# d-f/nylon-amt

Measured on AMD Instinct MI355X. Metric: training clips/sec (128-frame x 256-bin), higher is better.
Workload: dtype f16x3 (split fp16 / bf16 operand pairs, three bf16-rate MFMA passes per product, fp32 accumulate; tensors that flow between kernels are fp32 (attention q/k/v as fp16 hi+lo pairs), the copies SAVED only for the backward -- FFN hidden, its gradient, pre-LayerNorm sums -- are bf16); 1 GPU; paper-size hFT-Transformer training step (d=256, ff=512, 3+3 layers, 4 heads), batch 8 clips/GPU, dropout 0.10, forward+loss+backward+Adam; global_batch=8, frames=128, bins=256, parallelism=dp1, precision_mode=x3

## Files before the change

include/hftt_hip.h:

```cpp
#ifndef HFTT_HIP_H
#define HFTT_HIP_H
#include <stdint.h>
#ifdef __cplusplus
extern "C" {
#endif

#define HFTT_ABI_VERSION 8

int hftt_abi_version(void);
int hftt_build_options(void);
const char* hftt_last_error(void);
int hftt_device_cus(void);


typedef struct {
  int64_t src_off;
  int64_t dst_off;
  int32_t rows, cols, src_ld, dst_ld;
  int32_t kind;
  int32_t pad;
} hftt_prep_entry;
int hftt_prep_weights(const float* params, uint16_t* wbf, float* wf32, float* fdst,
                      const hftt_prep_entry* table_dev, int n_entries, void* stream);
int hftt_prep_weights_x3(const float* params, uint16_t* whi, uint16_t* wlo, float* fdst,
// ... 150 lines not shown
  float* dr; float* dr_drop;
  float drop_p; uint32_t drop_site; uint64_t drop_seed;
  float* ws;
  uint32_t drop_bf16;
  uint32_t io_flags;
} hftt_ln_bwd_desc;
#define HFTT_LNB_DY_BF16 1u
#define HFTT_LNB_DR_BF16 2u
#define HFTT_LNB_R_BF16 4u
int32_t hftt_ln_bwd_wgs(int32_t M);
int hftt_ln_bwd(const hftt_ln_bwd_desc* d, void* stream);
int hftt_ln_bwd_reduce(const float* ws, int32_t n_wg, int32_t N, float* dgamma, float* dbeta, float beta, void* stream);

#define HFTT_TE_X_BF16 1u
#define HFTT_TE_Y_BF16 2u
#define HFTT_TE_M_BF16 4u
int hftt_time_embed_fwd(const float* x, const float* pos, float* y, int32_t B, int32_t T, int32_t Nn, int32_t d,
                        float scale, float drop_p, uint32_t site, uint64_t seed, uint32_t io_flags, void* stream);
int hftt_time_embed_bwd(const float* dy, float* dx, float* dym, int32_t B, int32_t T, int32_t Nn, int32_t d,
                        float scale, float drop_p, uint32_t site, uint64_t seed, int32_t accumulate, uint32_t io_flags, void* stream);
int hftt_dropout_bwd(float* g, int64_t n, float drop_p, uint32_t site, uint64_t seed, uint32_t bf16, void* stream);
int hftt_colsum(const float* x, int64_t rows, int64_t n, int64_t ld, float* out, float beta, float* ws, uint32_t x_bf16, void* stream);
int64_t hftt_colsum_ws_bytes(int64_t rows, int64_t n);
int hftt_heads_split(const float* logits, int64_t ldl, float* onset, float* offset, float* mpe, float* velocity,
                     int32_t B, int32_t T, int32_t Nn, int32_t V, int32_t time_major, void* stream);
int hftt_heads_split_bwd(const float* p_onset, const float* p_offset, const float* p_mpe,
                         const float* d_onset, const float* d_offset, const float* d_mpe, const float* d_velocity,
                         float* dlogits, int64_t ldl, int32_t B, int32_t T, int32_t Nn, int32_t V, int32_t time_major,
                         void* stream);

typedef struct {
  int64_t n;
  int32_t V; int32_t pad;
  const float* prob[6];
  const float* vel[2];
  const float* label_onset; const float* label_offset; const float* label_mpe; const int64_t* label_velocity;
  float weight_A, weight_B, grad_scale; float pad2;
  float* d_prob[6]; float* d_vel[2];
  float* loss_out;
  float* ws;
} hftt_loss_desc;
int64_t hftt_loss_ws_bytes(int64_t n);
int hftt_loss(const hftt_loss_desc* d, void* stream);

int hftt_adam_step(float* p, const float* g, float* m, float* v, int64_t n, int32_t step,
                   double lr, double beta1, double beta2, double eps, double grad_scale, void* stream);
// ... 237 lines not shown
```

nylon-amt_amd/csrc/elementwise.hip:

```cpp
#include "hftt_common.h"
#include "x3_common.h"
#include "hftt_launch.h"
#include "../../include/hftt_hip.h"
#include <math.h>

namespace {

template <int E>
__device__ __forceinline__ void x3_split1(float x, uint16_t& hi, uint16_t& lo) {
  unsigned h, l;
  x3_split2_checked<E>(x, 0.f, h, l);
  hi = (uint16_t)(h & 0xFFFFu); lo = (uint16_t)(l & 0xFFFFu);
}

__global__ void prep_weights_kernel(const float* __restrict__ params, uint16_t* __restrict__ wbf, float* __restrict__ wf32,
                                    float* __restrict__ fdst, const hftt_prep_entry* __restrict__ table) {
  const hftt_prep_entry e = table[blockIdx.x];
  const long total = (long)e.rows * e.cols;
  for (long i = (long)blockIdx.y * blockDim.x + threadIdx.x; i < total; i += (long)gridDim.y * blockDim.x) {
    const int r = (int)(i / e.cols), c = (int)(i % e.cols);
    const float x = params[e.src_off + (long)r * e.src_ld + c];
    if (e.kind == 2) {
      fdst[e.dst_off + (long)r * e.dst_ld + c] = x;
    } else {
// ... 514 lines not shown
  for (long i = (long)blockIdx.x * blockDim.x + threadIdx.x; i < n4; i += (long)gridDim.x * blockDim.x) {
    const float4 a = hftt_load4(gbuf, bf, i * 4);
    float v[4] = {a.x, a.y, a.z, a.w};
    const uint32_t k4 = hftt_keep_quad(seed, site, (uint64_t)i, thr);
#pragma unroll
    for (int e = 0; e < 4; e++) v[e] = ((k4 >> e) & 1u) ? v[e] * inv_keep : 0.f;
    hftt_store4(gbuf, bf, i * 4, v[0], v[1], v[2], v[3]);
  }
}

constexpr int CS_SPLITS = 16;
__global__ void colsum_stage1_kernel(const float* __restrict__ x, long rows, long n, long ld, float* __restrict__ ws, uint32_t bf) {
  const long j = (long)blockIdx.x * blockDim.x + threadIdx.x;
  if (j >= n) return;
  const int sp = blockIdx.y;
  const long per = (rows + CS_SPLITS - 1) / CS_SPLITS;
  const long r0 = sp * per;
  long r1 = r0 + per; if (r1 > rows) r1 = rows;
  float acc = 0.f;
  if (bf) { for (long r = r0; r < r1; r++) acc += bf2f(reinterpret_cast<const unsigned short*>(x)[r * ld + j]); }
  else { for (long r = r0; r < r1; r++) acc += x[r * ld + j]; }
  ws[(long)sp * n + j] = acc;
}
__global__ void colsum_stage2_kernel(const float* __restrict__ ws, long n, float* __restrict__ out, float beta) {
  const long j = (long)blockIdx.x * blockDim.x + threadIdx.x;
  if (j >= n) return;
  float acc = 0.f;
#pragma unroll
  for (int s = 0; s < CS_SPLITS; s++) acc += ws[(long)s * n + j];
  out[j] = (beta != 0.f) ? (out[j] * beta + acc) : acc;
}

__device__ __forceinline__ float sigmoidf_(float x) { return 1.0f / (1.0f + expf(-x)); }

__global__ void heads_split_kernel(const float* __restrict__ logits, long ldl, float* __restrict__ onset, float* __restrict__ offset,
                                   float* __restrict__ mpe, float* __restrict__ velocity, int B, int T, int Nn, int V, int time_major) {
  const int v4 = V / 4;
  const long total = (long)B * T * Nn * v4;
  for (long i = (long)blockIdx.x * blockDim.x + threadIdx.x; i < total; i += (long)gridDim.x * blockDim.x) {
    const int c4 = (int)(i % v4);
    const long s = i / v4;
    long o = s;
    if (time_major) {
      const int t = (int)(s % T);
      const int n = (int)((s / T) % Nn);
      const int b = (int)(s / ((long)T * Nn));
// ... 276 lines not shown
  return hftt_launch<ln_bwd_reduce_kernel>("ln_bwd_reduce", dim3((2 * N + 15) / 16), dim3(256), 0, (hipStream_t)stream, ws, n_wg, N, dgamma, dbeta, beta);
}

extern "C" int hftt_time_embed_fwd(const float* x, const float* pos, float* y, int32_t B, int32_t T, int32_t Nn, int32_t d,
                                   float scale, float drop_p, uint32_t site, uint64_t seed, uint32_t io_flags, void* stream) {
  HFTT_REQUIRE(x && pos && y && d % 4 == 0, "time_embed_fwd: bad arguments");
  return hftt_launch<time_embed_fwd_kernel>("time_embed_fwd", dim3(grid_for((long)B * T * Nn * (d / 4), 256, 8192)), dim3(256), 0, (hipStream_t)stream,
                                                              x, pos, y, B, T, Nn, d, scale, drop_p, site, seed, io_flags);
}
extern "C" int hftt_time_embed_bwd(const float* dy, float* dx, float* dym, int32_t B, int32_t T, int32_t Nn, int32_t d,
                                   float scale, float drop_p, uint32_t site, uint64_t seed, int32_t accumulate, uint32_t io_flags, void* stream) {
  HFTT_REQUIRE(dy && dx && d % 4 == 0, "time_embed_bwd: bad arguments");
  return hftt_launch<time_embed_bwd_kernel>("time_embed_bwd", dim3(grid_for((long)B * T * Nn * (d / 4), 256, 8192)), dim3(256), 0, (hipStream_t)stream,
                                                              dy, dx, dym, B, T, Nn, d, scale, drop_p, site, seed, accumulate, io_flags);
}
extern "C" int hftt_dropout_bwd(float* g, int64_t n, float drop_p, uint32_t site, uint64_t seed, uint32_t bf16, void* stream) {
  HFTT_REQUIRE(g && n > 0 && n % 4 == 0 && drop_p >= 0.f && drop_p < 1.f && ((uintptr_t)g & 15) == 0, "dropout_bwd: bad arguments (n %% 4 == 0, 16-byte aligned)");
  if (drop_p == 0.f) return 0;
  return hftt_launch<dropout_bwd_kernel>("dropout_bwd", dim3(grid_for(n / 4, 256, 8192)), dim3(256), 0, (hipStream_t)stream, g, (long)n, drop_p, site, seed, bf16);
}
extern "C" int64_t hftt_colsum_ws_bytes(int64_t rows, int64_t n) { (void)rows; return (int64_t)CS_SPLITS * n * 4; }
extern "C" int hftt_colsum(const float* x, int64_t rows, int64_t n, int64_t ld, float* out, float beta, float* ws, uint32_t x_bf16, void* stream) {
  HFTT_REQUIRE(x && out && ws && rows > 0 && n > 0 && ld >= n, "colsum: bad arguments");
  if (int rc = hftt_launch<colsum_stage1_kernel>("colsum(1)", dim3((unsigned)((n + 255) / 256), CS_SPLITS), dim3(256), 0, (hipStream_t)stream, x, (long)rows, (long)n, (long)ld, ws, x_bf16)) return rc;
  return hftt_launch<colsum_stage2_kernel>("colsum(2)", dim3((unsigned)((n + 255) / 256)), dim3(256), 0, (hipStream_t)stream, ws, (long)n, out, beta);
}
extern "C" int hftt_heads_split(const float* logits, int64_t ldl, float* onset, float* offset, float* mpe, float* velocity,
                                int32_t B, int32_t T, int32_t Nn, int32_t V, int32_t time_major, void* stream) {
  HFTT_REQUIRE(logits && onset && offset && mpe && velocity, "heads_split: null operand");
  HFTT_REQUIRE(V % 4 == 0 && ldl % 4 == 0 && ldl >= V + 3, "heads_split: V=%d / ldl=%ld unsupported", V, (long)ldl);
  return hftt_launch<heads_split_kernel>("heads_split", dim3(grid_for((long)B * T * Nn * (V / 4), 256, 8192)), dim3(256), 0, (hipStream_t)stream,
                                                        logits, (long)ldl, onset, offset, mpe, velocity, B, T, Nn, V, time_major);
}
extern "C" int hftt_heads_split_bwd(const float* p_onset, const float* p_offset, const float* p_mpe,
                                    const float* d_onset, const float* d_offset, const float* d_mpe, const float* d_velocity,
                                    float* dlogits, int64_t ldl, int32_t B, int32_t T, int32_t Nn, int32_t V, int32_t time_major, void* stream) {
  HFTT_REQUIRE(p_onset && p_offset && p_mpe && d_onset && d_offset && d_mpe && d_velocity && dlogits, "heads_split_bwd: null operand");
  HFTT_REQUIRE(V % 4 == 0 && ldl % 4 == 0 && ldl >= V + 4, "heads_split_bwd: V=%d / ldl=%ld unsupported", V, (long)ldl);
  return hftt_launch<heads_split_bwd_kernel>("heads_split_bwd", dim3(grid_for((long)B * T * Nn * (ldl / 4), 256, 8192)), dim3(256), 0, (hipStream_t)stream,
                                                                p_onset, p_offset, p_mpe, d_onset, d_offset, d_mpe, d_velocity, dlogits, (long)ldl, B, T, Nn, V, time_major);
}

extern "C" int64_t hftt_loss_ws_bytes(int64_t n) { (void)n; return (int64_t)LOSS_WGS * 8 * 4; }
extern "C" int hftt_loss(const hftt_loss_desc* d, void* stream) {
  HFTT_REQUIRE(d && d->n > 0 && d->V > 0 && d->V <= 256, "loss: bad shape");
  for (int i = 0; i < 6; i++) HFTT_REQUIRE(d->prob[i] != nullptr, "loss: null probability tensor %d", i);
  HFTT_REQUIRE(d->vel[0] && d->vel[1] && d->label_onset && d->label_offset && d->label_mpe && d->label_velocity && d->loss_out && d->ws, "loss: null operand");
  int wgs = (int)((d->n + 3) / 4);
// ... 20 lines not shown
```

nylon-amt_amd/csrc/gemm_nt.hip:

```cpp
#include <type_traits>
#include "hftt_common.h"
#include "x3_common.h"
#include "hftt_launch.h"
#include "../../include/hftt_hip.h"

namespace {

__device__ __forceinline__ float4 load_gate4(const float* gate, bool bf, long off) {
  if (bf) {
    const uint2 u = *reinterpret_cast<const uint2*>(reinterpret_cast<const unsigned short*>(gate) + off);
    return make_float4(bf2f(u.x & 0xFFFFu), bf2f(u.x >> 16), bf2f(u.y & 0xFFFFu), bf2f(u.y >> 16));
  }
  return *reinterpret_cast<const float4*>(gate + off);
}
__device__ __forceinline__ void store_c4(float* C, bool bf, long off, float a, float b, float c, float d) {
  if (bf) {
    uint2 u;
    u.x = f2bf(a) | ((unsigned)f2bf(b) << 16); u.y = f2bf(c) | ((unsigned)f2bf(d) << 16);
    *reinterpret_cast<uint2*>(reinterpret_cast<unsigned short*>(C) + off) = u;
  } else {
    *reinterpret_cast<float4*>(C + off) = make_float4(a, b, c, d);
  }
}

// ... 371 lines not shown
      float s = 0.f;
#pragma unroll
      for (int e = 0; e < VPL; e++) s += v[e];
      const float mean = wave_sum(s) * (1.0f / BN);
      float q = 0.f;
#pragma unroll
      for (int e = 0; e < VPL; e++) { const float dlt = v[e] - mean; q += dlt * dlt; }
      const float var = wave_sum(q) * (1.0f / BN);
      const float rstd = 1.0f / sqrtf(var + 1e-5f);
#pragma unroll
      for (int e = 0; e < VPL; e++) {
        const int col = lane * VPL + e;
        if (g.pre_ln_out != nullptr) g.pre_ln_out[row * g.ldc + col] = v[e];
        g.C[row * g.ldc + col] = (v[e] - mean) * rstd * g.ln_gamma[col] + g.ln_beta[col];
      }
      if (lane == 0) {
        if (g.ln_mean != nullptr) g.ln_mean[row] = mean;
        if (g.ln_rstd != nullptr) g.ln_rstd[row] = rstd;
      }
    }
  }
}

template <int BM_, typename CH>
__device__ __forceinline__ void load_a_block(const hftt_gemm_nt_desc g, const long m0, unsigned short* As, const int RSA) {
  constexpr bool ABF = std::is_same<CH, uint4>::value;
  using T = typename std::conditional<ABF, unsigned short, float>::type;
  constexpr int E = 16 / sizeof(T);
  const T* A = reinterpret_cast<const T*>(g.A);
  const int cpr = g.K / E;
  const int total = BM_ * cpr;
  const int drow = 512 / cpr, dch = 512 - drow * cpr;
  int row = threadIdx.x / cpr, ch = threadIdx.x - row * cpr;
  for (int base = 0; base < total; base += 512 * 8) {
    CH v[8];
    int rr[8], cc[8];
#pragma unroll
    for (int u = 0; u < 8; u++) {
      rr[u] = row; cc[u] = ch;
      const bool in = row < BM_;
      const long grow = m0 + row;
      const long gr = (in && grow < g.M) ? grow : (m0 < g.M ? m0 : 0);
      const CH t = *reinterpret_cast<const CH*>(A + gr * g.lda + ch * E);
      if constexpr (ABF) v[u] = (in && grow < g.M) ? t : make_uint4(0u, 0u, 0u, 0u);
      else v[u] = (in && grow < g.M) ? t : make_float4(0.f, 0.f, 0.f, 0.f);
      row += drow; ch += dch;
      if (ch >= cpr) { ch -= cpr; row++; }
    }
#pragma unroll
    for (int u = 0; u < 8; u++)
      if (rr[u] < BM_) {
        unsigned short* dst = ABF ? As + rr[u] * RSA + (cc[u] << 3) : As + rr[u] * RSA + ((cc[u] >> 1) << 3) + (cc[u] & 1) * 4;
        if constexpr (ABF) {
          *reinterpret_cast<uint4*>(dst) = v[u];
        } else {
          typedef __bf16 bf4_t __attribute__((ext_vector_type(4)));
          const f32x4 fv = {v[u].x, v[u].y, v[u].z, v[u].w};
          *reinterpret_cast<uint2*>(dst) = __builtin_bit_cast(uint2, __builtin_convertvector(fv, bf4_t));
        }
      }
  }
}

template <int BM_, int MODE, bool EW = false, int PF = 1>
__global__ __launch_bounds__(512) __attribute__((amdgpu_waves_per_eu(4, MODE == 0 ? 8 : 4))) void gemm_nt_as1_kernel(const hftt_gemm_nt_desc g) {
  constexpr int BN = 256;
  constexpr int WM = (BM_ == 32) ? 1 : 2;
  constexpr int WN = 8 / WM;
  constexpr int TN = BN / (32 * WN);
  static_assert(BM_ == 32 * WM, "one 32-row MFMA tile per wave row");
  constexpr int RSW = 40;
  constexpr int W_ELEMS = BN * RSW;
  constexpr int WCH = 2;
  constexpr int STAGE_LD = BN + 4;
  static_assert(MODE != 2 || BM_ * STAGE_LD * 4 <= 2 * W_ELEMS * 2, "stage must fit the weight ring");
  extern __shared__ __attribute__((aligned(16))) unsigned char smem[];
  const int K = g.K;
  const int RSA = K + 8;
  unsigned short* As = reinterpret_cast<unsigned short*>(smem);
  unsigned short* Ws = As + BM_ * RSA;
  float* stage = (MODE == 2) ? reinterpret_cast<float*>(Ws) : reinterpret_cast<float*>(smem);

  const int tid = threadIdx.x, lane = tid & 63, wave = tid >> 6;
// ... 147 lines not shown
          const float v = fmaxf(acc[j][r] + bv, lo_clamp) * g.out_scale;
          acc[j][r] = 0.f;
          if (MODE != 0) {
            sp[rofs * STAGE_LD] = v;
          } else {
            if (full || m0 + rb0 + rofs < g.M) cp[(long)rofs * g.ldc] = v;
          }
        }
      }
      if (MODE != 0) {
        __syncthreads();
        row_pass<BM_ / 8, (BM_ / 8 < 4 ? BM_ / 8 : 4), true, true>(g, m0, n0, stage, STAGE_LD, true, thr, inv_keep);
        if (s + 1 < steps) {
          __syncthreads();
          wstore(wr[0], buf ^ 1);
        }
      }
    }
    __syncthreads();
    s++;
  }
}

template <int BM_, int MODE, bool EW = false, int PF = 1>
int launch_nt_as1(const hftt_gemm_nt_desc& d, hipStream_t st) {
  int lds = (BM_ * (d.K + 8) + 2 * 256 * 40) * 2;
  const int stage = BM_ * 260 * 4;
  if (MODE == 1 && stage > lds) lds = stage;
  dim3 grid((unsigned)((d.M + BM_ - 1) / BM_), 1, 1);
  return hftt_launch<gemm_nt_as1_kernel<BM_, MODE, EW, PF>>("gemm_nt", grid, dim3(512), lds, st, d);
}

template <int BN, int PREC, bool LN>
int launch_nt(const hftt_gemm_nt_desc& d, hipStream_t st) {
  using Cfg = NtCfg<BN, PREC>;
  int lds = Cfg::LOOP_BYTES;
  if ((LN || (Cfg::X3M && BN == 256)) && Cfg::STAGE_BYTES > lds) lds = Cfg::STAGE_BYTES;
  const int n_pad = ((d.N + 63) / 64) * 64;
  dim3 grid((unsigned)((d.M + BM - 1) / BM), (unsigned)((n_pad + BN - 1) / BN), 1);
  return hftt_launch<gemm_nt_kernel<BN, PREC, LN>>("gemm_nt", grid, dim3(512), lds, st, d);
}

template <int PREC>
int dispatch_nt(const hftt_gemm_nt_desc& d, hipStream_t st) {
  const int n_pad = ((d.N + 63) / 64) * 64;
  if (d.ln_gamma != nullptr) {
// ... 39 lines not shown
  return dispatch_nt<1>(d, st);
}

}

extern "C" int hftt_gemm_nt(const hftt_gemm_nt_desc* d, void* stream) {
  HFTT_REQUIRE(d != nullptr, "gemm_nt: null descriptor");
  HFTT_REQUIRE(d->M > 0 && d->N > 0 && d->K > 0, "gemm_nt: bad shape M=%d N=%d K=%d", d->M, d->N, d->K);
  HFTT_REQUIRE(d->K % 32 == 0, "gemm_nt: K=%d must be a multiple of 32", d->K);
  HFTT_REQUIRE((d->io_flags & ~HFTT_NT_A_HI) == 0 || d->npass == 1, "gemm_nt: bf16-stored operands need npass == 1");
  HFTT_REQUIRE(!(d->io_flags & HFTT_NT_A_HI) || d->npass == 4, "gemm_nt: HFTT_NT_A_HI goes with npass == 4");
  HFTT_REQUIRE(!(d->io_flags & HFTT_NT_C_BF16) || d->ln_gamma == nullptr, "gemm_nt: a bf16 C cannot be combined with LayerNorm");
  HFTT_REQUIRE(d->lda % ((d->io_flags & HFTT_NT_A_BF16) ? 8 : 4) == 0, "gemm_nt: lda=%ld breaks 16-byte row alignment", (long)d->lda);
  HFTT_REQUIRE(((uintptr_t)d->A & 15) == 0 && ((uintptr_t)d->W & 15) == 0, "gemm_nt: A/W must be 16-byte aligned");
  HFTT_REQUIRE(d->npass >= 1 && d->npass <= 4, "gemm_nt: npass must be 1 (bf16), 2 (split fp16), 3 (fp32) or 4 (split bf16)");
  HFTT_REQUIRE((d->npass != 2 && d->npass != 4) || d->W_lo != nullptr, "gemm_nt: the split modes need the lo weight plane (W_lo)");
  HFTT_REQUIRE(d->A != nullptr && d->W != nullptr && d->C != nullptr, "gemm_nt: null operand");
  HFTT_REQUIRE(d->add_table == nullptr || d->add_mod > 0, "gemm_nt: add_mod must be > 0");
  HFTT_REQUIRE(d->residual == nullptr || d->res_mod > 0, "gemm_nt: res_mod must be > 0");
  HFTT_REQUIRE(d->drop_p >= 0.f && d->drop_p < 1.f, "gemm_nt: drop_p out of range");
  HFTT_REQUIRE(d->ln_gamma == nullptr || (d->ln_beta != nullptr && d->ldc == d->N), "gemm_nt: LN needs beta and ldc == N");
  hipStream_t st = reinterpret_cast<hipStream_t>(stream);
  if (d->npass == 3) return dispatch_nt<3>(*d, st);
  if (d->npass == 2) return dispatch_nt<2>(*d, st);
#ifdef HFTT_GRAD_HI_BUILD
  if (d->npass == 4 && (d->io_flags & HFTT_NT_A_HI)) return dispatch_nt<5>(*d, st);
#else
  HFTT_REQUIRE(!(d->io_flags & HFTT_NT_A_HI), "gemm_nt: this library was built without the gradient-rounding option (HFTT_BUILD_GRAD_HI=1 python nylon-amt_amd/build.py)");
#endif
  if (d->npass == 4) return dispatch_nt<4>(*d, st);
  return dispatch_nt_bf16(*d, st);
}
```

nylon-amt_amd/hftt_hip/_capi.py:

```python
from __future__ import annotations

import ctypes as C
import os

_HERE = os.path.dirname(os.path.abspath(__file__))
_LIB_NAME = 'libhftt_hip_g' if os.environ.get('HFTT_BUILD_GRAD_HI') == '1' else 'libhftt_hip'
LIB_PATH = os.environ.get('HFTT_LIB_PATH') or os.path.join(_HERE, '..', 'lib', _LIB_NAME + '.so')

c_f32p = C.c_void_p
c_u16p = C.c_void_p


class PrepEntry(C.Structure):
    _fields_ = [('src_off', C.c_int64), ('dst_off', C.c_int64),
                ('rows', C.c_int32), ('cols', C.c_int32), ('src_ld', C.c_int32), ('dst_ld', C.c_int32),
                ('kind', C.c_int32), ('pad', C.c_int32)]


class GemmNtDesc(C.Structure):
    _fields_ = [('M', C.c_int32), ('N', C.c_int32), ('K', C.c_int32), ('npass', C.c_int32),
                ('A', c_f32p), ('lda', C.c_int64),
                ('W', C.c_void_p), ('io_flags', C.c_uint32), ('debug', C.c_uint32),
                ('bias', c_f32p),
                ('C', c_f32p), ('ldc', C.c_int64),
# ... 271 lines not shown
    'hftt_x3_strip_pack': (C.c_int, [c_f32p, c_u16p, C.c_void_p, C.c_int, C.c_int, C.c_void_p]),
    'hftt_strip_linear': (C.c_int, [C.POINTER(StripDesc), C.c_void_p]),
    'hftt_ffn_res_ln_fwd': (C.c_int, [C.POINTER(FfnDesc), C.c_void_p]),
    'hftt_ffn_bwd_dx': (C.c_int, [C.POINTER(FfnDesc), C.c_void_p]),
    'hftt_attn_out_ffn_fwd': (C.c_int, [C.POINTER(StripDesc), C.POINTER(FfnDesc), C.c_void_p]),
    'hftt_gemm_tn_ws_bytes': (C.c_int64, [C.c_int32, C.c_int32, C.c_int32]),
    'hftt_gemm_tn': (C.c_int, [C.POINTER(GemmTnDesc), C.c_void_p]),
    'hftt_attn_fwd': (C.c_int, [C.POINTER(AttnDesc), C.c_void_p]),
    'hftt_attn_bwd': (C.c_int, [C.POINTER(AttnDesc), C.c_void_p]),
    'hftt_x3_to_planes': (C.c_int, [c_f32p, C.c_int64, c_f32p, C.c_int64, C.c_int32, C.c_int32, C.c_void_p]),
    'hftt_embed_fold_fwd': (C.c_int, [C.POINTER(FoldDesc), C.c_void_p]),
    'hftt_embed_fold_bwd': (C.c_int, [C.POINTER(FoldDesc), C.c_void_p]),
    'hftt_im2win': (C.c_int, [c_f32p, c_f32p, C.c_int32, C.c_int32, C.c_int32, C.c_int32, C.c_int32, C.c_void_p]),
    'hftt_ln_bwd_wgs': (C.c_int32, [C.c_int32]),
    'hftt_ln_bwd': (C.c_int, [C.POINTER(LnBwdDesc), C.c_void_p]),
    'hftt_ln_bwd_reduce': (C.c_int, [c_f32p, C.c_int32, C.c_int32, c_f32p, c_f32p, C.c_float, C.c_void_p]),
    'hftt_time_embed_fwd': (C.c_int, [c_f32p, c_f32p, c_f32p, C.c_int32, C.c_int32, C.c_int32, C.c_int32,
                                      C.c_float, C.c_float, C.c_uint32, C.c_uint64, C.c_uint32, C.c_void_p]),
    'hftt_time_embed_bwd': (C.c_int, [c_f32p, c_f32p, c_f32p, C.c_int32, C.c_int32, C.c_int32, C.c_int32,
                                      C.c_float, C.c_float, C.c_uint32, C.c_uint64, C.c_int32, C.c_uint32, C.c_void_p]),
    'hftt_dropout_bwd': (C.c_int, [c_f32p, C.c_int64, C.c_float, C.c_uint32, C.c_uint64, C.c_uint32, C.c_void_p]),
    'hftt_colsum': (C.c_int, [c_f32p, C.c_int64, C.c_int64, C.c_int64, c_f32p, C.c_float, c_f32p, C.c_uint32, C.c_void_p]),
    'hftt_colsum_ws_bytes': (C.c_int64, [C.c_int64, C.c_int64]),
    'hftt_heads_split': (C.c_int, [c_f32p, C.c_int64, c_f32p, c_f32p, c_f32p, c_f32p,
                                   C.c_int32, C.c_int32, C.c_int32, C.c_int32, C.c_int32, C.c_void_p]),
    'hftt_heads_split_bwd': (C.c_int, [c_f32p, c_f32p, c_f32p, c_f32p, c_f32p, c_f32p, c_f32p, c_f32p, C.c_int64,
                                       C.c_int32, C.c_int32, C.c_int32, C.c_int32, C.c_int32, C.c_void_p]),
    'hftt_loss_ws_bytes': (C.c_int64, [C.c_int64]),
    'hftt_loss': (C.c_int, [C.POINTER(LossDesc), C.c_void_p]),
    'hftt_adam_step': (C.c_int, [c_f32p, c_f32p, c_f32p, c_f32p, C.c_int64, C.c_int32,
                                 C.c_double, C.c_double, C.c_double, C.c_double, C.c_double, C.c_void_p]),
    'hftt_logmel': (C.c_int, [C.POINTER(LogmelDesc), C.c_void_p]),
    'hftt_resample': (C.c_int, [C.POINTER(ResampleDesc), C.c_void_p]),
    'hftt_stitch': (C.c_int, [C.POINTER(StitchDesc), C.c_void_p]),
    'hftt_notes_ws_bytes': (C.c_int64, [C.c_int64, C.c_int32]),
    'hftt_notes_decode': (C.c_int, [C.POINTER(NotesDesc), C.c_void_p]),
    'hftt_clip_windows': (C.c_int, [C.POINTER(ClipWindowsDesc), C.c_void_p]),
    'hftt_notes_seg_ws_bytes': (C.c_int64, [C.c_int64, C.c_int32, C.c_int32]),
    'hftt_notes_decode_seg': (C.c_int, [C.POINTER(NotesSegDesc), C.c_void_p]),
    'hftt_notes_stream_state_bytes': (C.c_int64, [C.c_int32, C.c_int32]),
    'hftt_notes_stream_step': (C.c_int, [C.POINTER(NotesStreamDesc), C.c_void_p]),
    'hftt_labels_render': (C.c_int, [C.POINTER(LabelsDesc), C.c_void_p]),
    'hftt_clip_logmel': (C.c_int, [C.POINTER(ClipLogmelDesc), C.c_void_p]),
    'hftt_clip_logmel_warp': (C.c_int, [C.POINTER(ClipLogmelWarpDesc), C.c_void_p]),
    'hftt_wave_warp': (C.c_int, [C.POINTER(WaveWarpDesc), C.c_void_p]),
    'hftt_labels_render_warp': (C.c_int, [C.POINTER(LabelsWarpDesc), C.c_void_p]),
# ... 43 lines not shown
```

nylon-amt_amd/hftt_hip/engine.py:

```python
from __future__ import annotations

import ctypes as C
import math
import os

import torch

from . import _capi
from ._capi import FoldDesc, LossDesc, PrepEntry, StripPackEntry, check, lib
from .layout import PRECISION_NPASS, Options, WeightLayout, _align, flat_offsets, model_dims, precision_modes
from .plan import PlanBuilder, attn_fwd8_takes


def keep_scale(p):
    if not p > 0.0:
        return 1.0
    import numpy as np
    kk = (1.0 - float(np.float32(p))) * 256.0 + 0.5
    thr = 256 if kk >= 256.0 else (0 if kk <= 0.0 else int(kk))
    return float(np.float32(256.0) / np.float32(thr)) if thr > 0 else 0.0


def _table(entry_type, rows):
    return torch.frombuffer(bytearray(bytes((entry_type * len(rows))(*[entry_type(*r) for r in rows]))), dtype=torch.uint8)
# ... 210 lines not shown
            elif fn == 'heads':
                logits, tm = args
                o = outs[5:9] if tm else outs[0:4]
                rc = L.hftt_heads_split(logits, self.NHp, o[0].data_ptr(), o[1].data_ptr(), o[2].data_ptr(), o[3].data_ptr(), B, T, N, V, tm, stream)
            elif fn == 'heads_bwd':
                side, dlog, tm = args
                b = ws['bufs']
                po = outs[5:8] if tm else outs[0:3]
                rc = L.hftt_heads_split_bwd(po[0].data_ptr(), po[1].data_ptr(), po[2].data_ptr(),
                                            b['d.onset_' + side].data_ptr(), b['d.offset_' + side].data_ptr(), b['d.mpe_' + side].data_ptr(),
                                            b['d.velocity_' + side].data_ptr(), dlog, self.NHp, B, T, N, V, tm, stream)
            elif fn == 'time_embed':
                x, pos, y, site, iof = args
                rc = L.hftt_time_embed_fwd(x, pos, y, B, T, N, d, math.sqrt(d), p, site, seed, iof, stream)
            elif fn == 'time_embed_bwd':
                dy, dx, dym, site, iof = args
                rc = L.hftt_time_embed_bwd(dy, dx, dym, B, T, N, d, math.sqrt(d), p, site, seed, 1, iof, stream)
            elif fn == 'colsum':
                x, rows, n, ld, out, beta, wsp, xbf = args
                rc = L.hftt_colsum(x, rows, n, ld, out, beta, wsp, xbf, stream)
            elif fn == 'dropout_bwd':
                g, n, site, gbf = args
                rc = L.hftt_dropout_bwd(g, n, p, site, seed, gbf, stream) if p > 0.0 else 0
            else:
                raise _capi.HfttError('unknown plan op %s' % fn)
            if prof is not None:
                prof.end()
            if rc != 0:
                check(rc, name)

    def _patch(self, ws, p, seed):
        inv_keep = keep_scale(p)
        for dsc in ws['drop']:
            dsc.drop_p = p
            dsc.drop_seed = seed
        for dsc in ws.get('gate_descs', ()):
            dsc.gate_scale = inv_keep

    def forward(self, spec, training=False, outputs=None, save=None):
        if spec.dim() != 3 or spec.shape[1] != self.F or spec.shape[2] != self.W:
            raise _capi.HfttError('input_spec must be [B, %d, %d], got %s' % (self.F, self.W, tuple(spec.shape)))
        if not self.is_bound():
            raise _capi.HfttError('engine parameters are not bound (call bind first)')
        B = spec.shape[0]
        with torch.cuda.device(self.device):
            return self._forward(spec, B, training, outputs, save)
# ... 104 lines not shown
```

nylon-amt_amd/hftt_hip/plan.py:

```python
import ctypes as C
import math
import os

import torch

from . import _capi
from ._capi import (AttnDesc, FfnDesc, GemmNtDesc, GemmTnDesc, LnBwdDesc, StripDesc,
                    SL_C_BF16, SL_C_F16PAIR, SL_H_BF16, SL_PRE_BF16, SL_RELU, SL_X3_GRAD_HI, SL_RES_BF16, SL_X_BF16, SL_X3_F16, SL_X3_BF16, SL_X_DROP,
                    ATTN_Q_F16PAIR, ATTN_KV_F16PAIR)
from .layout import _align, qkv_planes


def attn_fwd8_takes(npass, hb, dh, Lq, Lk, probs):
    return (hb and dh == 64 and npass == 1 and 128 < Lk <= 256 and 128 < Lq <= 256 and not probs
            and os.environ.get('HFTT_ATTN_FWD8', '1')[:1] != '0')


def _tf(v):
    return 'true' if v else 'false'


def _env_on(name):
    return os.environ.get(name, '1')[:1] != '0'

# ... 3 lines not shown
    bn = N if ln else (256 if n_pad % 256 == 0 else (128 if n_pad % 128 == 0 else 64))
    esz = 2 if npass == 1 else 4
    nbytes = (2 if a_bf else 4) * M * K + (2 if c_bf else 4) * M * N + esz * N * K + ((2 if res_bf else 4) * M * N if residual else 0) + (4 * M * N if ln else 0) \
        + ((2 if gate_bf else 4) * M * N if gate else 0)
    rich = bool(add_table or gate or drop_site or residual or ln)
    if npass == 1 and N % 256 == 0 and K <= 768 and M >= 256:
        pf = 2 if (K // 32) % 2 == 0 else 1
        if K <= 256:
            elementwise = not (add_table or residual or ln) and c_bf and (not gate or gate_bf)
            if not rich:
                kname = 'gemm_nt_as1_kernel<64, 0, false, %d>' % pf
            elif elementwise:
                kname = 'gemm_nt_as1_kernel<64, 0, true, %d>' % pf
            elif N == 256:
                kname = 'gemm_nt_as1_kernel<64, 1, false, %d>' % pf
            else:
                kname = 'gemm_nt_as1_kernel<32, 2, false, 1>'
        elif N == 256 and K > 512:
            kname = 'gemm_nt_as1_kernel<64, 1, false, %d>' % pf
        elif N == 256 and pf == 2:
            kname = 'gemm_nt_as1_kernel<%d, 1, false, 2>' % (32 if ln else 64)
        else:
            kname = 'gemm_nt_as1_kernel<32, 2, false, 1>'
    else:
        kname = 'gemm_nt_kernel<%d, %d, %s>' % (bn, 5 if a_hi else npass, _tf(ln))
    return {'kernel': kname, 'flops': 2.0 * M * N * K, 'bytes': float(nbytes), 'shape': (M, N, K)}


def sl_meta(x3, small, hh, g8, backward, M, N, K, ln, pre_saved, residual, gate, c_planes, x_drop):
    bf = not x3
    nbytes = (2 if bf else 4) * M * K + (2 if bf else 4) * M * N + ((2 if (bf or hh) else 4) * M * N if pre_saved else 0) + (4 if x3 else 2) * N * K \
        + ((2 if bf else 4) * M * N if residual else 0) + (2 * M * N if gate else 0)
    passes, kch = N // 256, K // 256
    if small:
        kname = ('x3s_linear_kernel<%d, %d, %d, %s, %s>' % (4 if backward else 2, K // 32, N // 32, _tf(ln), _tf(residual))) if x3 \
            else 'bs_linear_kernel<%d, %d, %s, %s>' % (K // 32, N // 32, _tf(ln), _tf(residual))
    elif x3:
        xe = (5 if g8 else 4) if backward else 2
        if not ln and kch == 1:
            kname = 'x3_linear_n_kernel<%d, %d, %s, %s, %s>' % (xe, N // 32, _tf(residual), _tf(c_planes), _tf(x_drop))
        else:
            kname = 'x3_linear_kernel<%d, %s, %d, %d, %s, %d>' % (xe, _tf(ln), passes, kch, _tf(residual), 8 if (not ln and passes == 1) else 16)
    elif (_env_on('HFTT_STRIP_V2') and K % 256 == 0 and M % 32 == 0 and not gate
          and ((ln and kch <= 3) or (not ln and (kch, passes) in ((1, 1), (1, 2), (1, 3), (2, 1), (3, 1))))):
        kname = 'strip_linear2_kernel<%s, %d, %d, %s, %s>' % (_tf(ln), 1 if ln else passes, kch, _tf(residual), _tf(_env_on('HFTT_LINEAR2_PATCH')))
    else:
# ... 592 lines not shown
            else:
                self.tn(Se, 2 * d, d, eGq, 2 * d, enc, d, [(0, d, e.G(pc + 'fc_k.weight'), e.G(pc + 'fc_k.bias')), (d, d, e.G(pc + 'fc_v.weight'), e.G(pc + 'fc_v.bias'))])
                if enc_grad:
                    self.linear(Se, d, 2 * d, eGq, 2 * d, tag + '.ca.kv_t', 0, eGA, d, residual=0 if first_enc_grad else eGA,
                                ldr=d if (st or not first_enc_grad) else 0)
                first_enc_grad = False
            if j > 0:
                self.tn(Sn, d, d, Q1, d, b[tag + '.x1'].data_ptr(), d, [(0, d, e.G(pc + 'fc_q.weight'), e.G(pc + 'fc_q.bias'))])
                self.linear(Sn, d, d, Q1, d, tag + '.ca.q_t', 0, A, d, residual=Bf, ldr=d)
                self.self_attn_bwd(tag, pre, Sn, BT, N, H, ws['dec_out'][j - 1], Gd, sites['self'])
            else:
                gpos = e.G(dd + 'pos_embedding_freq.weight')
                plan.append(('colsum', (Bf, BT, N * d, N * d, gpos, 0.0, cs_ws, 1 if bs else 0), 'colsum', None))
                plan.append(('colsum', (q1f if bs else Q1, BT, N * d, N * d, dq0s, 0.0, cs_ws, 0), 'colsum', None))
                self.tn(N, d, d, dq0s, d, e.P(dd + 'pos_embedding_freq.weight'), d, [(0, d, e.G(pc + 'fc_q.weight'), e.G(pc + 'fc_q.bias'))])
                self.nt(N, d, d, dq0s, d, e.Wp(tag + '.ca.q_t'), 0, gpos, d, residual=gpos, ldr=d)
        marks.append((len(plan), o_dec, o_time))
        if not enc_grad:
            ws['bwd_dec'], ws['bwd_dec_marks'] = plan, marks
            return
        Ge = (eGA, eGB, eGC, eGh, eGq, eGx)
        for i in reversed(range(e.Le)):
            self.enc_layer_bwd(f'enc{i}', f'{enc_}layers_freq.{i}.', Se, BT, F, e.He, ws['enc_in'][i], Ge, dx_fp32=(i == 0))
        plan.append(('dropout_bwd', (eGA, Se * d, ws['sites']['embed'], 1 if bs else 0), 'dropout_bwd', None))
        plan.append(('colsum', (eGA, BT, F * d, F * d, e.G(enc_ + 'pos_embedding_freq.weight'), 0.0, cs_ws, 1 if bs else 0), 'colsum', None))
        self.tn(Se, d, e.Kp, eGA, d, b['win'].data_ptr(), e.Kp, [(0, d, e.dweff.data_ptr(), e.dbeff.data_ptr())], out_scale=math.sqrt(d))
        plan.append((self.lib.hftt_embed_fold_bwd, (C.byref(e.fold),), 'embed_fold_bwd', None))
        marks.append((len(plan), 0, o_dec))
        ws['bwd'] = plan
        ws['bwd_marks'] = marks
```

Before: 290.1 clips/s.

## Add persistent streamed x3 NT GEMM kernel and fuse dropout-backward with colsum

Adds a persistent gemm_nt_as3 kernel for npass 2/4 NT GEMMs with K<=256 and N up to 256, used by default unless HFTT_NT_STREAM=0. Each workgroup loops over row blocks and double-buffers the weight hi/lo tiles through registers and LDS, prefetching the next A block during the last k-step. The encoder embed dropout backward and positional-embedding column sum become one fused kernel, and the generic colsum gains a float4-vectorised row-batched stage 1. The aim is less launch and global-memory traffic and more load/compute overlap, at the cost of fixed waves-per-EU occupancy and more LDS per workgroup.

```diff
diff --git a/include/hftt_hip.h b/include/hftt_hip.h
--- a/include/hftt_hip.h
+++ b/include/hftt_hip.h
@@ -196,6 +196,8 @@
 int hftt_dropout_bwd(float* g, int64_t n, float drop_p, uint32_t site, uint64_t seed, uint32_t bf16, void* stream);
 int hftt_colsum(const float* x, int64_t rows, int64_t n, int64_t ld, float* out, float beta, float* ws, uint32_t x_bf16, void* stream);
 int64_t hftt_colsum_ws_bytes(int64_t rows, int64_t n);
+int hftt_dropout_bwd_colsum(float* g, int64_t rows, int64_t n, int64_t ld, float drop_p, uint32_t site, uint64_t seed, float* out, float beta,
+                            float* ws, uint32_t bf16, void* stream);
 int hftt_heads_split(const float* logits, int64_t ldl, float* onset, float* offset, float* mpe, float* velocity,
                      int32_t B, int32_t T, int32_t Nn, int32_t V, int32_t time_major, void* stream);
 int hftt_heads_split_bwd(const float* p_onset, const float* p_offset, const float* p_mpe,
diff --git a/nylon-amt_amd/csrc/elementwise.hip b/nylon-amt_amd/csrc/elementwise.hip
--- a/nylon-amt_amd/csrc/elementwise.hip
+++ b/nylon-amt_amd/csrc/elementwise.hip
@@ -560,6 +560,48 @@
   else { for (long r = r0; r < r1; r++) acc += x[r * ld + j]; }
   ws[(long)sp * n + j] = acc;
 }
+constexpr int DCS_RB = 8;
+__global__ __launch_bounds__(256) void dropout_bwd_colsum_stage1_kernel(float* gbuf, long rows, long n, long ld, float drop_p, uint32_t site, uint64_t seed,
+                                                                        float* __restrict__ ws, uint32_t bf) {
+  const long j = ((long)blockIdx.x * blockDim.x + threadIdx.x) * 4;
+  if (j >= n) return;
+  const uint32_t thr = hftt_keep_thr(drop_p);
+  const float inv_keep = hftt_keep_scale(drop_p);
+  const bool mask = drop_p > 0.f;
+  const int sp = blockIdx.y;
+  const long per = (rows + CS_SPLITS - 1) / CS_SPLITS;
+  const long r0 = sp * per;
+  long r1 = r0 + per; if (r1 > rows) r1 = rows;
+  float acc[4] = {0.f, 0.f, 0.f, 0.f};
+  for (long r = r0; r < r1; r += DCS_RB) {
+    float4 a[DCS_RB];
+#pragma unroll
+    for (int u = 0; u < DCS_RB; u++) {
+      const long rc = r + u < r1 ? r + u : r1 - 1;
+      a[u] = hftt_load4(gbuf, bf, rc * ld + j);
+    }
+#pragma unroll
+    for (int u = 0; u < DCS_RB; u++) {
+      if (r + u < r1) {
+        const long off = (r + u) * ld + j;
+        float v[4] = {a[u].x, a[u].y, a[u].z, a[u].w};
+        if (mask) {
+          const uint32_t k4 = hftt_keep_quad(seed, site, (uint64_t)off >> 2, thr);
+#pragma unroll
+          for (int e = 0; e < 4; e++) v[e] = ((k4 >> e) & 1u) ? __fmul_rn(v[e], inv_keep) : 0.f;
+          hftt_store4(gbuf, bf, off, v[0], v[1], v[2], v[3]);
+          if (bf) {
+#pragma unroll
+            for (int e = 0; e < 4; e++) v[e] = bf2f(f2bf(v[e]));
+          }
+        }
+#pragma unroll
+        for (int e = 0; e < 4; e++) acc[e] += v[e];
+      }
+    }
+  }
+  *reinterpret_cast<float4*>(ws + (long)sp * n + j) = make_float4(acc[0], acc[1], acc[2], acc[3]);
+}
 __global__ void colsum_stage2_kernel(const float* __restrict__ ws, long n, float* __restrict__ out, float beta) {
   const long j = (long)blockIdx.x * blockDim.x + threadIdx.x;
   if (j >= n) return;
@@ -882,8 +924,21 @@
 extern "C" int64_t hftt_colsum_ws_bytes(int64_t rows, int64_t n) { (void)rows; return (int64_t)CS_SPLITS * n * 4; }
 extern "C" int hftt_colsum(const float* x, int64_t rows, int64_t n, int64_t ld, float* out, float beta, float* ws, uint32_t x_bf16, void* stream) {
   HFTT_REQUIRE(x && out && ws && rows > 0 && n > 0 && ld >= n, "colsum: bad arguments");
+  if (n % 4 == 0 && ld % 4 == 0 && (((uintptr_t)x | (uintptr_t)ws) & 15) == 0) {
+    if (int rc = hftt_launch<dropout_bwd_colsum_stage1_kernel>("colsum(1)", dim3((unsigned)((n / 4 + 255) / 256), CS_SPLITS), dim3(256), 0, (hipStream_t)stream,
+                                                               const_cast<float*>(x), (long)rows, (long)n, (long)ld, 0.f, 0u, (uint64_t)0, ws, x_bf16)) return rc;
+    return hftt_launch<colsum_stage2_kernel>("colsum(2)", dim3((unsigned)((n + 255) / 256)), dim3(256), 0, (hipStream_t)stream, ws, (long)n, out, beta);
+  }
   if (int rc = hftt_launch<colsum_stage1_kernel>("colsum(1)", dim3((unsigned)((n + 255) / 256), CS_SPLITS), dim3(256), 0, (hipStream_t)stream, x, (long)rows, (long)n, (long)ld, ws, x_bf16)) return rc;
   return hftt_launch<colsum_stage2_kernel>("colsum(2)", dim3((unsigned)((n + 255) / 256)), dim3(256), 0, (hipStream_t)stream, ws, (long)n, out, beta);
+}
+extern "C" int hftt_dropout_bwd_colsum(float* g, int64_t rows, int64_t n, int64_t ld, float drop_p, uint32_t site, uint64_t seed, float* out, float beta,
+                                       float* ws, uint32_t bf16, void* stream) {
+  HFTT_REQUIRE(g && out && ws && rows > 0 && n > 0 && ld >= n && drop_p >= 0.f && drop_p < 1.f, "dropout_bwd_colsum: bad arguments");
+  HFTT_REQUIRE(n % 4 == 0 && ld % 4 == 0 && ((uintptr_t)g & 15) == 0 && ((uintptr_t)ws & 15) == 0, "dropout_bwd_colsum: n %% 4 == 0, ld %% 4 == 0, g and ws 16-byte aligned");
+  if (int rc = hftt_launch<dropout_bwd_colsum_stage1_kernel>("dropout_bwd_colsum(1)", dim3((unsigned)((n / 4 + 255) / 256), CS_SPLITS), dim3(256), 0, (hipStream_t)stream,
+                                                             g, (long)rows, (long)n, (long)ld, drop_p, site, seed, ws, bf16)) return rc;
+  return hftt_launch<colsum_stage2_kernel>("dropout_bwd_colsum(2)", dim3((unsigned)((n + 255) / 256)), dim3(256), 0, (hipStream_t)stream, ws, (long)n, out, beta);
 }
 extern "C" int hftt_heads_split(const float* logits, int64_t ldl, float* onset, float* offset, float* mpe, float* velocity,
                                 int32_t B, int32_t T, int32_t Nn, int32_t V, int32_t time_major, void* stream) {
diff --git a/nylon-amt_amd/csrc/gemm_nt.hip b/nylon-amt_amd/csrc/gemm_nt.hip
--- a/nylon-amt_amd/csrc/gemm_nt.hip
+++ b/nylon-amt_amd/csrc/gemm_nt.hip
@@ -1,3 +1,4 @@
+#include <cstdlib>
 #include <type_traits>
 #include "hftt_common.h"
 #include "x3_common.h"
@@ -417,43 +418,56 @@
   }
 }
 
-template <int BM_, typename CH>
-__device__ __forceinline__ void load_a_block(const hftt_gemm_nt_desc g, const long m0, unsigned short* As, const int RSA) {
+struct AWalk {
+  int cpr, drow, dch, row, ch;
+  __device__ __forceinline__ AWalk(int cpr_) : cpr(cpr_), drow(512 / cpr_), dch(512 - (512 / cpr_) * cpr_) {
+    row = threadIdx.x / cpr; ch = threadIdx.x - row * cpr;
+  }
+  __device__ __forceinline__ void next() {
+    row += drow; ch += dch;
+    if (ch >= cpr) { ch -= cpr; row++; }
+  }
+};
+template <int BM_, typename CH, int NCH>
+__device__ __forceinline__ void a_block_issue(const hftt_gemm_nt_desc& g, const long m0, AWalk& w, CH (&v)[NCH]) {
   constexpr bool ABF = std::is_same<CH, uint4>::value;
   using T = typename std::conditional<ABF, unsigned short, float>::type;
   constexpr int E = 16 / sizeof(T);
   const T* A = reinterpret_cast<const T*>(g.A);
-  const int cpr = g.K / E;
-  const int total = BM_ * cpr;
-  const int drow = 512 / cpr, dch = 512 - drow * cpr;
-  int row = threadIdx.x / cpr, ch = threadIdx.x - row * cpr;
+#pragma unroll
+  for (int u = 0; u < NCH; u++) {
+    const long grow = m0 + w.row;
+    const long gr = (w.row < BM_ && grow < g.M) ? grow : (m0 < g.M ? m0 : 0);
+    v[u] = *reinterpret_cast<const CH*>(A + gr * g.lda + w.ch * E);
+    w.next();
+  }
+}
+template <int BM_>
+__device__ __forceinline__ bool a_chunk_live(const hftt_gemm_nt_desc& g, const long m0, const AWalk& w) { return w.row < BM_ && m0 + w.row < g.M; }
+template <int BM_, typename CH>
+__device__ __forceinline__ void load_a_block(const hftt_gemm_nt_desc g, const long m0, unsigned short* As, const int RSA) {
+  constexpr bool ABF = std::is_same<CH, uint4>::value;
+  AWalk w(g.K / (ABF ? 8 : 4));
+  const int total = BM_ * w.cpr;
   for (int base = 0; base < total; base += 512 * 8) {
     CH v[8];
-    int rr[8], cc[8];
+    AWalk at = w;
+    a_block_issue<BM_, CH, 8>(g, m0, w, v);
 #pragma unroll
     for (int u = 0; u < 8; u++) {
-      rr[u] = row; cc[u] = ch;
-      const bool in = row < BM_;
-      const long grow = m0 + row;
-      const long gr = (in && grow < g.M) ? grow : (m0 < g.M ? m0 : 0);
-      const CH t = *reinterpret_cast<const CH*>(A + gr * g.lda + ch * E);
-      if constexpr (ABF) v[u] = (in && grow < g.M) ? t : make_uint4(0u, 0u, 0u, 0u);
-      else v[u] = (in && grow < g.M) ? t : make_float4(0.f, 0.f, 0.f, 0.f);
-      row += drow; ch += dch;
-      if (ch >= cpr) { ch -= cpr; row++; }
-    }
-#pragma unroll
-    for (int u = 0; u < 8; u++)
-      if (rr[u] < BM_) {
-        unsigned short* dst = ABF ? As + rr[u] * RSA + (cc[u] << 3) : As + rr[u] * RSA + ((cc[u] >> 1) << 3) + (cc[u] & 1) * 4;
+      if (at.row < BM_) {
+        unsigned short* dst = ABF ? As + at.row * RSA + (at.ch << 3) : As + at.row * RSA + ((at.ch >> 1) << 3) + (at.ch & 1) * 4;
+        const bool live = a_chunk_live<BM_>(g, m0, at);
         if constexpr (ABF) {
-          *reinterpret_cast<uint4*>(dst) = v[u];
+          *reinterpret_cast<uint4*>(dst) = live ? v[u] : make_uint4(0u, 0u, 0u, 0u);
         } else {
           typedef __bf16 bf4_t __attribute__((ext_vector_type(4)));
-          const f32x4 fv = {v[u].x, v[u].y, v[u].z, v[u].w};
+          const f32x4 fv = {live ? v[u].x : 0.f, live ? v[u].y : 0.f, live ? v[u].z : 0.f, live ? v[u].w : 0.f};
           *reinterpret_cast<uint2*>(dst) = __builtin_bit_cast(uint2, __builtin_convertvector(fv, bf4_t));
         }
       }
+      at.next();
+    }
   }
 }
 
@@ -647,6 +661,202 @@
   }
 }
 
+constexpr int AS3_BM = 64;
+constexpr int AS3_RSW = 40;
+constexpr int AS3_W_ELEMS = 2 * 256 * AS3_RSW;
+constexpr int AS3_STAGE_LD = 256 + 4;
+constexpr int as3_a_bytes(int nch) {
+  const int a = AS3_BM * (nch * 32 + 8) * 2 * 2, s = AS3_BM * AS3_STAGE_LD * 4;
+  return a > s ? a : s;
+}
+constexpr int as3_lds_bytes(int nch) { return as3_a_bytes(nch) + 2 * AS3_W_ELEMS * 2; }
+
+template <int XE, int NCH, bool PF2>
+__global__ __launch_bounds__(512) __attribute__((amdgpu_waves_per_eu(2, 2))) void gemm_nt_as3_kernel(const hftt_gemm_nt_desc g, const int nblk) {
+  constexpr int BM_ = AS3_BM, BN = 256, WN = 4, TN = 2, RSW = AS3_RSW, STAGE_LD = AS3_STAGE_LD;
+  extern __shared__ __attribute__((aligned(16))) unsigned char smem[];
+  const int K = g.K;
+  const int RSA = K + 8;
+  unsigned short* As = reinterpret_cast<unsigned short*>(smem);
+  unsigned short* Ws = reinterpret_cast<unsigned short*>(smem + as3_a_bytes(NCH));
+  float* stage = reinterpret_cast<float*>(smem);
+
+  const int tid = threadIdx.x, lane = tid & 63, wave = tid >> 6;
+  const int wm = wave / WN, wn = wave % WN;
+  const int lr = lane & 31, lh = lane >> 5;
+  const int KT = K / 32;
+  const unsigned short* Wb = reinterpret_cast<const unsigned short*>(g.W);
+  const unsigned short* Wlo = reinterpret_cast<const unsigned short*>(g.W_lo);
+
+  struct WRegs { uint4 h0, h1, l0, l1; };
+  const uint4 z4 = make_uint4(0u, 0u, 0u, 0u);
+  WRegs w0 = {z4, z4, z4, z4}, w1 = {z4, z4, z4, z4};
+  const int wrow = tid >> 2, wch = tid & 3;
+  const long wg0 = (long)(wrow < g.N ? wrow : g.N - 1) * K + wch * 8, wg1 = (long)(wrow + 128 < g.N ? wrow + 128 : g.N - 1) * K + wch * 8;
+  const int ws0 = wrow * RSW + wch * 8, ws1 = ws0 + 128 * RSW;
+  auto wload = [&](WRegs& w, int kt) __attribute__((always_inline)) {
+    w.h0 = *reinterpret_cast<const uint4*>(Wb + wg0 + kt * 32); w.h1 = *reinterpret_cast<const uint4*>(Wb + wg1 + kt * 32);
+    w.l0 = *reinterpret_cast<const uint4*>(Wlo + wg0 + kt * 32); w.l1 = *reinterpret_cast<const uint4*>(Wlo + wg1 + kt * 32);
+    __builtin_amdgcn_sched_barrier(0);
+  };
+  auto wstore = [&](const WRegs& w, int buf) __attribute__((always_inline)) {
+    unsigned short* d = Ws + buf * AS3_W_ELEMS;
+    *reinterpret_cast<uint4*>(d + ws0) = w.h0; *reinterpret_cast<uint4*>(d + ws1) = w.h1;
+    *reinterpret_cast<uint4*>(d + BN * RSW + ws0) = w.l0; *reinterpret_cast<uint4*>(d + BN * RSW + ws1) = w.l1;
+  };
+  float4 av[NCH];
+  auto a_issue = [&](long m0) __attribute__((always_inline)) {
+    AWalk w(K / 4);
+    a_block_issue<BM_, float4, NCH>(g, m0, w, av);
+    __builtin_amdgcn_sched_barrier(0);
+  };
+  auto a_commit = [&](long m0) __attribute__((always_inline)) {
+    AWalk w(K / 4);
+#pragma unroll
+    for (int u = 0; u < NCH; u++) {
+      if (w.row < BM_) {
+        uint2 hi, lo;
+        x3_split4<XE>(a_chunk_live<BM_>(g, m0, w) ? av[u] : make_float4(0.f, 0.f, 0.f, 0.f), hi, lo);
+        unsigned short* dst = As + w.row * RSA + w.ch * 4;
+        *reinterpret_cast<uint2*>(dst) = hi;
+        *reinterpret_cast<uint2*>(dst + BM_ * RSA) = lo;
+      }
+      w.next();
+    }
+  };
+
+  f32x16 acc[TN];
+  auto k_step = [&](int kt, int buf) __attribute__((always_inline)) {
+    const unsigned short* Wt = Ws + buf * AS3_W_ELEMS;
+#pragma unroll
+    for (int ks = 0; ks < 2; ks++) {
+      const unsigned short* pa = As + (wm * 32 + lr) * RSA + kt * 32 + ks * 16 + lh * 8;
+      const bf16x8 ah = lds_read_b128(pa), al = lds_read_b128(pa + BM_ * RSA);
+#pragma unroll
+      for (int j = 0; j < TN; j++) {
+        const unsigned short* pb = Wt + (wn * TN * 32 + j * 32 + lr) * RSW + ks * 16 + lh * 8;
+        const bf16x8 bh = lds_read_b128(pb), bl = lds_read_b128(pb + BN * RSW);
+        acc[j] = x3_mma<XE>(ah, al, bh, bl, acc[j]);
+      }
+    }
+  };
+
+  const uint32_t thr = hftt_keep_thr(g.drop_p);
+  const float inv_keep = hftt_keep_scale(g.drop_p);
+  const bool rowpass = (g.N % 4 == 0) && (g.gate == nullptr || g.ldg % 4 == 0) && (g.residual == nullptr || g.ldr % 4 == 0) &&
+                       ((((uintptr_t)g.gate | (uintptr_t)g.residual | (uintptr_t)g.add_table) & 15) == 0);
+
+  float bv[TN];
+#pragma unroll
+  for (int j = 0; j < TN; j++) {
+    const int col_l = wn * TN * 32 + j * 32 + lr;
+    bv[j] = (g.bias != nullptr && col_l < g.N) ? g.bias[col_l] : 0.f;
+  }
+  long blk = blockIdx.x;
+  wload(w0, 0);
+  if constexpr (PF2) wload(w1, 1);
+  a_issue(blk * BM_);
+  wstore(w0, 0);
+  int s = 0;
+  for (; blk < nblk; blk += gridDim.x) {
+    const long m0 = blk * BM_;
+    a_commit(m0);
+    __syncthreads();
+#pragma unroll
+    for (int j = 0; j < TN; j++)
+#pragma unroll
+      for (int r = 0; r < 16; r++) acc[j][r] = 0.f;
+    if constexpr (PF2) {
+      for (int kt = 0; kt + 2 < KT; kt += 2) {
+        wload(w0, kt + 2); k_step(kt, 0); wstore(w1, 1);
+        __syncthreads();
+        wload(w1, kt + 3); k_step(kt + 1, 1); wstore(w0, 0);
+        __syncthreads();
+      }
+      wload(w0, 0); k_step(KT - 2, 0); wstore(w1, 1);
+      __syncthreads();
+      wload(w1, 1);
+      a_issue((blk + gridDim.x) * BM_);
+      k_step(KT - 1, 1); wstore(w0, 0);
+      __syncthreads();
+    } else {
+      for (int kt = 0; kt + 1 < KT; kt++) {
+        wload(w0, kt + 1); k_step(kt, s & 1); wstore(w0, (s & 1) ^ 1);
+        __syncthreads();
+        s++;
+      }
+      wload(w0, 0);
+      a_issue((blk + gridDim.x) * BM_);
+      k_step(KT - 1, s & 1); wstore(w0, (s & 1) ^ 1);
+      __syncthreads();
+      s++;
+    }
+
+#pragma unroll
+    for (int j = 0; j < TN; j++) {
+      const int col_l = wn * TN * 32 + j * 32 + lr;
+#pragma unroll
+      for (int r = 0; r < 16; r++) {
+        const int row_l = wm * 32 + acc_row32(r, lh);
+        float v = acc[j][r] + bv[j];
+        if (g.act == 1) v = fmaxf(v, 0.f);
+        v *= g.out_scale;
+        stage[row_l * STAGE_LD + col_l] = v;
+      }
+    }
+    __syncthreads();
+    if (rowpass) {
+      row_pass<BM_ / 8, NCH == 4 ? 8 : 4, false, false>(g, m0, 0, stage, STAGE_LD, lane * 4 < g.N, thr, inv_keep);
+    } else {
+      const int c4 = lane * 4;
+#pragma unroll 1
+      for (int rr = 0; rr < BM_ / 8; rr++) {
+        const int row_l = wave * (BM_ / 8) + rr;
+        const long row = m0 + row_l;
+        if (row >= g.M) break;
+        const float4 sv = *reinterpret_cast<const float4*>(stage + row_l * STAGE_LD + c4);
+        float* cp = g.C + row * g.ldc + c4;
+        if (c4 + 4 <= g.N) {
+          *reinterpret_cast<float4*>(cp) = sv;
+        } else {
+          if (c4 < g.N) cp[0] = sv.x;
+          if (c4 + 1 < g.N) cp[1] = sv.y;
+          if (c4 + 2 < g.N) cp[2] = sv.z;
+        }
+      }
+    }
+    __syncthreads();
+  }
+}
+
+bool nt_as3_enabled() {
+  const char* e = getenv("HFTT_NT_STREAM");
+  return !(e != nullptr && e[0] == '0');
+}
+bool nt_as3_takes(const hftt_gemm_nt_desc& d) {
+  if (d.ln_gamma != nullptr || d.K > 256 || !(d.N == 256 || (d.K == 256 && d.N <= 256))) return false;
+  if (d.ldc % 4 != 0 || ((uintptr_t)d.C & 15) != 0) return false;
+  const bool rich = d.add_table || d.gate || d.drop_p > 0.f || d.residual;
+  const bool quads = (d.N % 4 == 0) && (!d.gate || d.ldg % 4 == 0) && (!d.residual || d.ldr % 4 == 0) &&
+                     ((((uintptr_t)d.gate | (uintptr_t)d.residual | (uintptr_t)d.add_table) & 15) == 0);
+  return (quads || !rich) && nt_as3_enabled();
+}
+template <int XE, int NCH, bool PF2>
+int launch_nt_as3(const hftt_gemm_nt_desc& d, hipStream_t st) {
+  constexpr int lds = as3_lds_bytes(NCH);
+  const int nblk = (d.M + AS3_BM - 1) / AS3_BM;
+  int wgs = 0;
+  if (int rc = hftt_resident_wgs<gemm_nt_as3_kernel<XE, NCH, PF2>>("gemm_nt", 512, lds, &wgs)) return rc;
+  dim3 grid((unsigned)(nblk < wgs ? nblk : wgs), 1, 1);
+  return hftt_launch<gemm_nt_as3_kernel<XE, NCH, PF2>>("gemm_nt", grid, dim3(512), lds, st, d, nblk);
+}
+template <int XE>
+int dispatch_nt_as3(const hftt_gemm_nt_desc& d, hipStream_t st) {
+  const bool pf2 = (d.K / 32) % 2 == 0;
+  if (d.K <= 128) return pf2 ? launch_nt_as3<XE, 4, true>(d, st) : launch_nt_as3<XE, 4, false>(d, st);
+  return pf2 ? launch_nt_as3<XE, 8, true>(d, st) : launch_nt_as3<XE, 8, false>(d, st);
+}
+
 template <int BM_, int MODE, bool EW = false, int PF = 1>
 int launch_nt_as1(const hftt_gemm_nt_desc& d, hipStream_t st) {
   int lds = (BM_ * (d.K + 8) + 2 * 256 * 40) * 2;
@@ -732,12 +942,12 @@
   HFTT_REQUIRE(d->ln_gamma == nullptr || (d->ln_beta != nullptr && d->ldc == d->N), "gemm_nt: LN needs beta and ldc == N");
   hipStream_t st = reinterpret_cast<hipStream_t>(stream);
   if (d->npass == 3) return dispatch_nt<3>(*d, st);
-  if (d->npass == 2) return dispatch_nt<2>(*d, st);
+  if (d->npass == 2) return nt_as3_takes(*d) ? dispatch_nt_as3<X3_F16>(*d, st) : dispatch_nt<2>(*d, st);
 #ifdef HFTT_GRAD_HI_BUILD
   if (d->npass == 4 && (d->io_flags & HFTT_NT_A_HI)) return dispatch_nt<5>(*d, st);
 #else
   HFTT_REQUIRE(!(d->io_flags & HFTT_NT_A_HI), "gemm_nt: this library was built without the gradient-rounding option (HFTT_BUILD_GRAD_HI=1 python nylon-amt_amd/build.py)");
 #endif
-  if (d->npass == 4) return dispatch_nt<4>(*d, st);
+  if (d->npass == 4) return nt_as3_takes(*d) ? dispatch_nt_as3<X3_BF16>(*d, st) : dispatch_nt<4>(*d, st);
   return dispatch_nt_bf16(*d, st);
 }
diff --git a/nylon-amt_amd/hftt_hip/_capi.py b/nylon-amt_amd/hftt_hip/_capi.py
--- a/nylon-amt_amd/hftt_hip/_capi.py
+++ b/nylon-amt_amd/hftt_hip/_capi.py
@@ -317,6 +317,8 @@
     'hftt_dropout_bwd': (C.c_int, [c_f32p, C.c_int64, C.c_float, C.c_uint32, C.c_uint64, C.c_uint32, C.c_void_p]),
     'hftt_colsum': (C.c_int, [c_f32p, C.c_int64, C.c_int64, C.c_int64, c_f32p, C.c_float, c_f32p, C.c_uint32, C.c_void_p]),
     'hftt_colsum_ws_bytes': (C.c_int64, [C.c_int64, C.c_int64]),
+    'hftt_dropout_bwd_colsum': (C.c_int, [c_f32p, C.c_int64, C.c_int64, C.c_int64, C.c_float, C.c_uint32, C.c_uint64, c_f32p, C.c_float, c_f32p,
+                                          C.c_uint32, C.c_void_p]),
     'hftt_heads_split': (C.c_int, [c_f32p, C.c_int64, c_f32p, c_f32p, c_f32p, c_f32p,
                                    C.c_int32, C.c_int32, C.c_int32, C.c_int32, C.c_int32, C.c_void_p]),
     'hftt_heads_split_bwd': (C.c_int, [c_f32p, c_f32p, c_f32p, c_f32p, c_f32p, c_f32p, c_f32p, c_f32p, C.c_int64,
diff --git a/nylon-amt_amd/hftt_hip/engine.py b/nylon-amt_amd/hftt_hip/engine.py
--- a/nylon-amt_amd/hftt_hip/engine.py
+++ b/nylon-amt_amd/hftt_hip/engine.py
@@ -256,6 +256,9 @@
             elif fn == 'dropout_bwd':
                 g, n, site, gbf = args
                 rc = L.hftt_dropout_bwd(g, n, p, site, seed, gbf, stream) if p > 0.0 else 0
+            elif fn == 'dropout_bwd_colsum':
+                g, rows, n, ld, site, out, beta, wsp, gbf = args
+                rc = L.hftt_dropout_bwd_colsum(g, rows, n, ld, p, site, seed, out, beta, wsp, gbf, stream)
             else:
                 raise _capi.HfttError('unknown plan op %s' % fn)
             if prof is not None:
diff --git a/nylon-amt_amd/hftt_hip/plan.py b/nylon-amt_amd/hftt_hip/plan.py
--- a/nylon-amt_amd/hftt_hip/plan.py
+++ b/nylon-amt_amd/hftt_hip/plan.py
@@ -49,6 +49,9 @@
             kname = 'gemm_nt_as1_kernel<%d, 1, false, 2>' % (32 if ln else 64)
         else:
             kname = 'gemm_nt_as1_kernel<32, 2, false, 1>'
+    elif (npass in (2, 4) and not a_hi and not ln and K <= 256 and (N == 256 or (K == 256 and N <= 256)) and (N % 4 == 0 or not rich)
+          and _env_on('HFTT_NT_STREAM')):
+        kname = 'gemm_nt_as3_kernel<%d, %d, %s>' % (npass, 4 if K <= 128 else 8, _tf((K // 32) % 2 == 0))
     else:
         kname = 'gemm_nt_kernel<%d, %d, %s>' % (bn, 5 if a_hi else npass, _tf(ln))
     return {'kernel': kname, 'flops': 2.0 * M * N * K, 'bytes': float(nbytes), 'shape': (M, N, K)}
@@ -687,8 +690,8 @@
         Ge = (eGA, eGB, eGC, eGh, eGq, eGx)
         for i in reversed(range(e.Le)):
             self.enc_layer_bwd(f'enc{i}', f'{enc_}layers_freq.{i}.', Se, BT, F, e.He, ws['enc_in'][i], Ge, dx_fp32=(i == 0))
-        plan.append(('dropout_bwd', (eGA, Se * d, ws['sites']['embed'], 1 if bs else 0), 'dropout_bwd', None))
-        plan.append(('colsum', (eGA, BT, F * d, F * d, e.G(enc_ + 'pos_embedding_freq.weight'), 0.0, cs_ws, 1 if bs else 0), 'colsum', None))
+        plan.append(('dropout_bwd_colsum', (eGA, BT, F * d, F * d, ws['sites']['embed'], e.G(enc_ + 'pos_embedding_freq.weight'), 0.0, cs_ws, 1 if bs else 0),
+                     'dropout_bwd_colsum', None))
         self.tn(Se, d, e.Kp, eGA, d, b['win'].data_ptr(), e.Kp, [(0, d, e.dweff.data_ptr(), e.dbeff.data_ptr())], out_scale=math.sqrt(d))
         plan.append((self.lib.hftt_embed_fold_bwd, (C.byref(e.fold),), 'embed_fold_bwd', None))
         marks.append((len(plan), 0, o_dec))
```

Result: faster. 294.6 clips/s, median of 6 (+1.6%).
